# flashlight/wav2letter

Hardware: NVIDIA H100
Metric: frames_per_sec (higher is better)
Workload: dtype f32

## Files before the change

### wav2letter_b200/csrc/am_kernels.cu

```cuda
#include <cuda_runtime.h>

#include <cooperative_groups.h>

#include "common.cuh"

namespace w2l {
bool conv_mma_supported(int W, int Cin, int Cout, int K, int stride);
size_t conv_mma_arranged_floats(int Cin, int Cout, int K);
int conv_mma_fwd(cudaStream_t stream, int B, int T, int Tout, int W, int Cin, int Cout, int K, int stride, int pad_left,
                 const float* x, const float* wt, int wt_cin, int wt_cout, int flip, const float* bias, const float* add, float* y,
                 int act, float drop_p, unsigned long long seed, float* arranged, int Kfull, int tap_step, int tap_off,
                 int out_fstride, int out_foff, int out_frames);
size_t conv_mma_wgrad_parts(int B, int Tout, int W, int Cin, int Cout, int K, int stride, int* tc_out, int* per_sample_out);
int conv_mma_wgrad(cudaStream_t stream, int B, int T, int Tout, int W, int Cin, int Cout, int K, int stride, int pad_left,
                   const float* x, const float* dy, float* dwt, float* dbias, float* partial);


namespace {

constexpr int kConvRows = 4;

template <int CO, int TT>
__global__ void __launch_bounds__(96 * kConvRows) conv_time_fwd_kernel(
    int T, int Tout, int W, int Cin, int Cout, int K, int stride, int pad_left, const float* __restrict__ x,
    const float* __restrict__ wt_arranged, const float* __restrict__ bias, const float* add,
    float* y, int act, float drop_p, unsigned long long seed) {
  extern __shared__ __align__(16) float wsm[];
  const int b = blockIdx.y;
  const int w = threadIdx.x;
  const int to0 = (blockIdx.x * kConvRows + threadIdx.y) * TT;
  const int nw = Cin * K * CO;
  for (int i = threadIdx.y * blockDim.x + threadIdx.x; i < nw; i += blockDim.x * blockDim.y) wsm[i] = wt_arranged[i];
  __syncthreads();
  if (w >= W || to0 >= Tout) return;
  float acc[TT][CO];
#pragma unroll
  for (int c = 0; c < CO; ++c) {
    const float bv = (bias != nullptr && c < Cout) ? __ldg(bias + c) : 0.f;
#pragma unroll
    for (int h = 0; h < TT; ++h) acc[h][c] = bv;
  }
  const float* xb = x + (size_t)b * T * Cin * W + w;
  const size_t tstride = (size_t)Cin * W;
  for (int ci = 0; ci < Cin; ++ci) {
    const float* xc = xb + (size_t)ci * W;
    const float* wrow = wsm + (size_t)ci * K * CO;
    for (int dk = 0; dk < K; ++dk) {
      float xv[TT];
#pragma unroll
      for (int h = 0; h < TT; ++h) {
        const int tin = (to0 + h) * stride + dk - pad_left;
        xv[h] = (tin >= 0 && tin < T) ? __ldg(xc + (size_t)tin * tstride) : 0.f;
      }
      const float4* w4 = reinterpret_cast<const float4*>(wrow + dk * CO);
#pragma unroll
      for (int q = 0; q < CO / 4; ++q) {
        const float4 wv = w4[q];
#pragma unroll
        for (int h = 0; h < TT; ++h) {
          acc[h][4 * q + 0] = fmaf(xv[h], wv.x, acc[h][4 * q + 0]);
          acc[h][4 * q + 1] = fmaf(xv[h], wv.y, acc[h][4 * q + 1]);
          acc[h][4 * q + 2] = fmaf(xv[h], wv.z, acc[h][4 * q + 2]);
          acc[h][4 * q + 3] = fmaf(xv[h], wv.w, acc[h][4 * q + 3]);
        }
      }
    }
  }
  const float inv_keep = drop_p > 0.f ? 1.0f / (1.0f - drop_p) : 1.0f;
#pragma unroll
  for (int h = 0; h < TT; ++h) {
    if (to0 + h >= Tout) continue;
#pragma unroll
    for (int c = 0; c < CO; ++c) {
      if (c < Cout) {
        const size_t idx = (((size_t)b * Tout + to0 + h) * Cout + c) * W + w;
        float v = acc[h][c];
        if (act == 1) v = fmaxf(v, 0.f);
        if (drop_p > 0.f) v *= dropout_scale(seed, idx, drop_p, inv_keep);
        if (add != nullptr) v += add[idx];
        y[idx] = v;
      }
    }
  }
}

__global__ void conv_arrange_weights_kernel(int Cin, int Cout, int K, int CO, const float* __restrict__ wt,
                                            float* __restrict__ out, int flip_for_dgrad) {
  const int n_out = (flip_for_dgrad ? Cout : Cin) * K * CO;
  for (int i = blockIdx.x * blockDim.x + threadIdx.x; i < n_out; i += gridDim.x * blockDim.x) {
    const int c_inner = i % CO, dk = (i / CO) % K, c_outer = i / (CO * K);
    float v = 0.f;
    if (!flip_for_dgrad) {
      if (c_inner < Cout) v = wt[((size_t)c_inner * Cin + c_outer) * K + dk];
    } else {
      if (c_inner < Cin) v = wt[((size_t)c_outer * Cin + c_inner) * K + (K - 1 - dk)];
    }
// ... 571 lines not shown
  __syncthreads();
  int b = 0;
  for (int i = threadIdx.x; i < n_loss; i += blockDim.x) b |= !isfinite(loss[i]);
  if (b) atomicOr(&bad_loss, 1);
  __syncthreads();
  if (threadIdx.x == 0) {
    const int bad = bad_norm | bad_loss, again = retry != nullptr && bad_norm && !bad_loss;
    guard[0] = bad;
    if (bad && !again) guard[1] += 1;
    if (retry != nullptr) *retry = again;
  }
}

struct BandMasks {
  int nf, nt;
  int f0[8], f1[8], t0[8], t1[8];
};
__global__ void __launch_bounds__(256) mask_bands_kernel(long long n, int W, int CW, int T, const float* __restrict__ x, float* __restrict__ y,
                                                         BandMasks m, float val) {
  for (long long i = (long long)blockIdx.x * blockDim.x + threadIdx.x; i < n; i += (long long)gridDim.x * blockDim.x) {
    const int w = (int)(i % W), t = (int)((i / CW) % T);
    bool hit = false;
#pragma unroll
    for (int k = 0; k < 8; ++k) hit = hit || (k < m.nf && w >= m.f0[k] && w < m.f1[k]) || (k < m.nt && t >= m.t0[k] && t < m.t1[k]);
    y[i] = hit ? val : x[i];
  }
}

__global__ void transpose_bft_kernel(int F, int T, const float* __restrict__ in, float* __restrict__ out) {
  __shared__ float tile[32][33];
  const int b = blockIdx.z;
  const int t0 = blockIdx.x * 32, f0 = blockIdx.y * 32;
  const float* ib = in + (size_t)b * F * T;
  float* ob = out + (size_t)b * T * F;
  for (int j = threadIdx.y; j < 32; j += blockDim.y) {
    const int f = f0 + j, t = t0 + threadIdx.x;
    tile[j][threadIdx.x] = (f < F && t < T) ? ib[(size_t)f * T + t] : 0.f;
  }
  __syncthreads();
  for (int j = threadIdx.y; j < 32; j += blockDim.y) {
    const int t = t0 + j, f = f0 + threadIdx.x;
    if (t < T && f < F) ob[(size_t)t * F + f] = tile[threadIdx.x][j];
  }
}
template <int V>
__global__ void axpy_kernel(long long n, float a, const float* __restrict__ x, float* __restrict__ y) {
  const long long start = V * ((long long)blockIdx.x * blockDim.x + threadIdx.x), step = V * (long long)gridDim.x * blockDim.x;
#pragma unroll 2
  for (long long i = start; i < n; i += step) stv<V>(y, i, vmap([&](float xv, float yv) { return fmaf(a, xv, yv); }, ldv<V>(x, i), ldv<V>(y, i)));
}
__global__ void fill_kernel(long long n, float v, float* __restrict__ y) {
  for (long long i = (long long)blockIdx.x * blockDim.x + threadIdx.x; i < n; i += (long long)gridDim.x * blockDim.x) y[i] = v;
}
__global__ void mask_mul_kernel(long long n, const float* __restrict__ g, const float* __restrict__ ref, int mode, float scale,
                                float* __restrict__ out) {
  for (long long i = (long long)blockIdx.x * blockDim.x + threadIdx.x; i < n; i += (long long)gridDim.x * blockDim.x) {
    const float r = ref[i];
    out[i] = ((mode == 1 ? r > 0.f : r != 0.f) ? scale : 0.f) * g[i];
  }
}
__global__ void act_fwd_kernel(long long n, const float* __restrict__ x, int relu, float drop_p, unsigned long long seed,
                               float* __restrict__ y) {
  const float inv_keep = drop_p > 0.f ? 1.0f / (1.0f - drop_p) : 1.0f;
  for (long long i = (long long)blockIdx.x * blockDim.x + threadIdx.x; i < n; i += (long long)gridDim.x * blockDim.x) {
    float v = x[i];
    if (relu) v = fmaxf(v, 0.f);
    if (drop_p > 0.f) v *= dropout_scale(seed, (unsigned long long)i, drop_p, inv_keep);
    y[i] = v;
  }
}

int blocks_for(long long n, int per_block = 256 * 8) { return (int)std::min<long long>((n + per_block - 1) / per_block, sm_count() * 8); }

}
}

using namespace w2l;

static int co_pad(int c) { return (c + 3) / 4 * 4; }

static size_t conv_ws_partial_bytes(int B, int Tout, int Cin, int Cout, int K) {
  const size_t per = ((size_t)Cout * Cin * K + Cout) * sizeof(float);
  const size_t simt = (size_t)B * ((Tout + 15) / 16);
  const size_t mma = conv_mma_wgrad_parts(B, Tout, 0, Cin, Cout, K, 1, nullptr, nullptr);
  return align_up(std::max(simt, std::max(mma, (size_t)B * (size_t)std::max(Tout, 16))) * per, 256);
}
extern "C" size_t w2l_conv_time_workspace_size(int B, int Tout, int Cin, int Cout, int K) {
  const size_t arranged =
      std::max((size_t)std::max(Cin, Cout) * K * co_pad(std::max(Cin, Cout)), conv_mma_arranged_floats(Cin, Cout, K)) * sizeof(float);
  return conv_ws_partial_bytes(B, Tout, Cin, Cout, K) + align_up(arranged, 256);
}

#define W2L_CONV_DISPATCH(CO_VAL, ...)                   \
  switch (CO_VAL) {                                              \
    case 4: { constexpr int CO = 4; constexpr int TT = 8; (void)TT; __VA_ARGS__; } break;        \
    case 8: { constexpr int CO = 8; constexpr int TT = 8; (void)TT; __VA_ARGS__; } break;        \
    case 12: { constexpr int CO = 12; constexpr int TT = 8; (void)TT; __VA_ARGS__; } break;      \
    case 16: { constexpr int CO = 16; constexpr int TT = 6; (void)TT; __VA_ARGS__; } break;      \
    case 20: { constexpr int CO = 20; constexpr int TT = 4; (void)TT; __VA_ARGS__; } break;      \
    case 24: { constexpr int CO = 24; constexpr int TT = 4; (void)TT; __VA_ARGS__; } break;      \
    case 28: { constexpr int CO = 28; constexpr int TT = 3; (void)TT; __VA_ARGS__; } break;      \
    case 32: { constexpr int CO = 32; constexpr int TT = 3; (void)TT; __VA_ARGS__; } break;      \
    default: return fail(W2L_ERR_UNSUPPORTED, "conv_time: more than 32 channels is not covered"); \
  }

static int conv_check(int B, int T, int Tout, int W, int Cin, int Cout, int K, int stride) {
  if (B <= 0 || T <= 0 || Tout <= 0 || W <= 0 || Cin <= 0 || Cout <= 0 || K <= 0 || stride <= 0)
    return fail(W2L_ERR_INVALID_ARGUMENT, "conv_time: non-positive dimension");
  if (W > 80) return fail(W2L_ERR_UNSUPPORTED, "conv_time: W > 80 is not covered");
  if (Cin > 32 || Cout > 32) return fail(W2L_ERR_UNSUPPORTED, "conv_time: more than 32 channels is not covered");
  return W2L_OK;
}

extern "C" int w2l_conv_time_fwd(void* stream_, int B, int T, int Tout, int W, int Cin, int Cout, int K, int stride,
                                 int pad_left, const float* x, const float* wt, const float* bias, const float* add,
                                 float* y, int act, float dropout_p, unsigned long long seed, void* ws, size_t ws_bytes) {
  cudaStream_t stream = static_cast<cudaStream_t>(stream_);
  if (int rc = conv_check(B, T, Tout, W, Cin, Cout, K, stride)) return rc;
  if (!x || !wt || !y || !ws) return fail(W2L_ERR_INVALID_ARGUMENT, "conv_time_fwd: null pointer");
  if (ws_bytes < w2l_conv_time_workspace_size(B, Tout, Cin, Cout, K)) return fail(W2L_ERR_WORKSPACE, "conv_time_fwd: workspace too small");
  const int CO = co_pad(Cout);
  float* arranged = reinterpret_cast<float*>(static_cast<char*>(ws) + conv_ws_partial_bytes(B, Tout, Cin, Cout, K));
  if (conv_mma_supported(W, Cin, Cout, K, stride))
    return conv_mma_fwd(stream, B, T, Tout, W, Cin, Cout, K, stride, pad_left, x, wt, Cin, Cout, 0, bias, add, y, act, dropout_p, seed,
                        arranged, K, 1, 0, 1, 0, Tout);
  conv_arrange_weights_kernel<<<8, 256, 0, stream>>>(Cin, Cout, K, CO, wt, arranged, 0);
  W2L_LAUNCH_CHECK("conv_arrange_weights_kernel");
  const size_t smem = (size_t)Cin * K * CO * sizeof(float);
  dim3 block(96, kConvRows);
  W2L_CONV_DISPATCH(CO, {
    if (smem > 48 * 1024)
      W2L_CUDA_CHECK(cudaFuncSetAttribute(conv_time_fwd_kernel<CO, TT>, cudaFuncAttributeMaxDynamicSharedMemorySize, (int)smem));
    dim3 grid((Tout + kConvRows * TT - 1) / (kConvRows * TT), B);
    conv_time_fwd_kernel<CO, TT><<<grid, block, smem, stream>>>(T, Tout, W, Cin, Cout, K, stride, pad_left, x, arranged, bias, add,
                                                                y, act, dropout_p, seed);
  });
  W2L_LAUNCH_CHECK("conv_time_fwd_kernel");
  return W2L_OK;
}

extern "C" int w2l_conv_time_dgrad(void* stream_, int B, int T, int Tout, int W, int Cin, int Cout, int K, int stride,
                                   int pad_left, const float* dy, const float* wt, const float* add, float* dx, void* ws,
                                   size_t ws_bytes) {
  cudaStream_t stream = static_cast<cudaStream_t>(stream_);
  if (int rc = conv_check(B, T, Tout, W, Cin, Cout, K, stride)) return rc;
  if (!dy || !wt || !dx || !ws) return fail(W2L_ERR_INVALID_ARGUMENT, "conv_time_dgrad: null pointer");
  if (ws_bytes < w2l_conv_time_workspace_size(B, Tout, Cin, Cout, K)) return fail(W2L_ERR_WORKSPACE, "conv_time_dgrad: workspace too small");
  if (stride == 1 && conv_mma_supported(W, Cout, Cin, K, 1)) {
    float* arranged = reinterpret_cast<float*>(static_cast<char*>(ws) + conv_ws_partial_bytes(B, Tout, Cin, Cout, K));
    return conv_mma_fwd(stream, B, Tout, T, W, Cout, Cin, K, 1, K - 1 - pad_left, dy, wt, Cin, Cout, 1, nullptr, add, dx, 0, 0.f, 0ull,
                        arranged, K, 1, 0, 1, 0, T);
  }
  if (stride > 1 && stride <= K && conv_mma_supported(W, Cout, Cin, (K + stride - 1) / stride, 1)) {
    float* arranged = reinterpret_cast<float*>(static_cast<char*>(ws) + conv_ws_partial_bytes(B, Tout, Cin, Cout, K));
    for (int p = 0; p < stride; ++p) {
      const int Kp = (K - p + stride - 1) / stride;
      const int d = pad_left - p;
      const int u_min = d > 0 ? (d + stride - 1) / stride : 0;
      const int t0 = stride * u_min + p - pad_left;
      const int n_u = t0 < T ? (T - 1 - t0) / stride + 1 : 0;
      if (n_u <= 0) continue;
      if (int rc = conv_mma_fwd(stream, B, Tout, n_u, W, Cout, Cin, Kp, 1, Kp - 1 - u_min, dy, wt, Cin, Cout, 1, nullptr, add, dx, 0, 0.f, 0ull,
                                arranged, K, stride, p, stride, t0, T))
        return rc;
    }
    return W2L_OK;
  }
  if (stride == 1 && Tout == T) {
// ... 286 lines not shown
```

### wav2letter_b200/csrc/conv_mma.cu

```cuda
#include <cuda_runtime.h>

#include "common.cuh"

namespace w2l {
namespace {

constexpr int kMmaThreads = 256;

__device__ __forceinline__ float to_tf32(float x) {
  uint32_t r;
  asm("cvt.rna.tf32.f32 %0, %1;" : "=r"(r) : "f"(x));
  return __uint_as_float(r);
}
__device__ __forceinline__ float rn_tf32(float x) { return __uint_as_float((__float_as_uint(x) + 0x1000u) & 0xffffe000u); }
__device__ __forceinline__ void split_tf32(float x, float& hi, float& lo) {
  hi = rn_tf32(x);
  lo = rn_tf32(x - hi);
}
__device__ __forceinline__ void mma_tf32(float (&d)[4], const float (&a)[4], const float (&b)[2]) {
  asm volatile(
      "mma.sync.aligned.m16n8k8.row.col.f32.tf32.tf32.f32 {%0,%1,%2,%3}, {%4,%5,%6,%7}, {%8,%9}, {%0,%1,%2,%3};"
      : "+f"(d[0]), "+f"(d[1]), "+f"(d[2]), "+f"(d[3])
      : "r"(__float_as_uint(a[0])), "r"(__float_as_uint(a[1])), "r"(__float_as_uint(a[2])), "r"(__float_as_uint(a[3])),
        "r"(__float_as_uint(b[0])), "r"(__float_as_uint(b[1])));
}
template <int WT, bool kRaw = false>
__device__ __forceinline__ void stage_rows(float* dst, int pitch, const float* __restrict__ src, int W, int row_base,
                                           int rows_total, int nrows, int zero_rows) {
  constexpr int q = 2 * WT, RPW = 32 / q, kWarps = kMmaThreads / 32;
  const int warp = threadIdx.x >> 5, lane = threadIdx.x & 31;
  const int sub = lane / q, c4 = lane % q;
  if (sub < RPW) {
#pragma unroll 4
    for (int r = warp * RPW + sub; r < nrows; r += kWarps * RPW) {
      const int gr = r + row_base;
      float4 v = make_float4(0.f, 0.f, 0.f, 0.f);
      if (gr >= 0 && gr < rows_total) v = __ldg(reinterpret_cast<const float4*>(src + (size_t)gr * W) + c4);
      *reinterpret_cast<float4*>(dst + (size_t)r * pitch + 4 * c4) = kRaw ? v : make_float4(to_tf32(v.x), to_tf32(v.y), to_tf32(v.z), to_tf32(v.w));
    }
  }
  for (int i = threadIdx.x; i < zero_rows * pitch; i += blockDim.x) dst[(size_t)nrows * pitch + i] = 0.f;
}

__host__ __device__ constexpr int fwd_pitch(int WT) { return (8 * WT) % 16 == 8 ? 8 * WT : 8 * WT + 8; }
__host__ __device__ constexpr int wg_pitch(int WT) { return 8 * WT + 4; }

template <int MT, int UPW, int WT, bool kX3>
__global__ void __launch_bounds__(kMmaThreads, 2) conv_mma_fwd_kernel(int T, int Tout, int W, int Cin, int Cout, int K, int stride,
                                                                       int pad_left, int Kpad, int apitch,
                                                                       const float* __restrict__ x, const float* __restrict__ wa,
                                                                       const float* __restrict__ bias, const float* add,
                                                                       float* y, int act, float drop_p,
                                                                       unsigned long long seed, int out_fstride, int out_foff,
                                                                       int out_frames) {
  extern __shared__ __align__(16) float sm[];
  constexpr int kPitch = fwd_pitch(WT);
  constexpr int TB = 8 * UPW;
  float* xs = sm;
  const int b = blockIdx.z, w_off = blockIdx.y * 8 * WT, to0 = blockIdx.x * TB;
  const int nto = min(TB, Tout - to0);
  const int warp = threadIdx.x >> 5, lane = threadIdx.x & 31, g = lane >> 2, t4 = lane & 3;
  float acc[UPW][MT][WT][4];
#pragma unroll
  for (int u = 0; u < UPW; ++u)
#pragma unroll
    for (int m = 0; m < MT; ++m)
#pragma unroll
      for (int j = 0; j < WT; ++j)
#pragma unroll
        for (int q = 0; q < 4; ++q) acc[u][m][j][q] = 0.f;
  const int nframes = (nto - 1) * stride + K;
  stage_rows<WT, kX3>(xs, kPitch, x + (size_t)b * T * Cin * W + w_off, W, (to0 * stride - pad_left) * Cin, T * Cin, nframes * Cin, 8);
  __syncthreads();
  const float* bp[UPW];
#pragma unroll
  for (int u = 0; u < UPW; ++u) bp[u] = xs + (size_t)(min(warp + 8 * u, nto - 1) * stride * Cin + t4) * kPitch + g;
  const float* ap = wa + (size_t)g * apitch + t4;
  float a[MT][4];
#pragma unroll
  for (int m = 0; m < MT; ++m) {
    a[m][0] = __ldg(ap + (size_t)16 * m * apitch);
    a[m][1] = __ldg(ap + (size_t)(16 * m + 8) * apitch);
    a[m][2] = __ldg(ap + (size_t)16 * m * apitch + 4);
    a[m][3] = __ldg(ap + (size_t)(16 * m + 8) * apitch + 4);
  }
  for (int k0 = 0; k0 < Kpad; k0 += 8) {
    float an[MT][4];
    const int kn = min(k0 + 8, Kpad - 8);
#pragma unroll
    for (int m = 0; m < MT; ++m) {
      an[m][0] = __ldg(ap + (size_t)16 * m * apitch + kn);
      an[m][1] = __ldg(ap + (size_t)(16 * m + 8) * apitch + kn);
      an[m][2] = __ldg(ap + (size_t)16 * m * apitch + kn + 4);
      an[m][3] = __ldg(ap + (size_t)(16 * m + 8) * apitch + kn + 4);
    }
    float ah[MT][4], al[MT][4];
    if (kX3) {
#pragma unroll
      for (int m = 0; m < MT; ++m)
#pragma unroll
        for (int q = 0; q < 4; ++q) split_tf32(a[m][q], ah[m][q], al[m][q]);
    }
#pragma unroll
    for (int u = 0; u < UPW; ++u) {
      const float* bq = bp[u] + (size_t)k0 * kPitch;
#pragma unroll
      for (int j = 0; j < WT; ++j) {
        float bf[2];
        bf[0] = bq[8 * j];
        bf[1] = bq[4 * kPitch + 8 * j];
        if (kX3) {
          float bh[2], bl[2];
          split_tf32(bf[0], bh[0], bl[0]);
          split_tf32(bf[1], bh[1], bl[1]);
#pragma unroll
          for (int m = 0; m < MT; ++m) {
            mma_tf32(acc[u][m][j], al[m], bh);
            mma_tf32(acc[u][m][j], ah[m], bl);
            mma_tf32(acc[u][m][j], ah[m], bh);
          }
        } else {
#pragma unroll
          for (int m = 0; m < MT; ++m) mma_tf32(acc[u][m][j], a[m], bf);
        }
      }
    }
#pragma unroll
    for (int m = 0; m < MT; ++m)
#pragma unroll
      for (int q = 0; q < 4; ++q) a[m][q] = an[m][q];
  }
  const float inv_keep = drop_p > 0.f ? 1.0f / (1.0f - drop_p) : 1.0f;
  const bool odd = t4 & 1;
#pragma unroll
  for (int u = 0; u < UPW; ++u) {
    const int tl = warp + 8 * u;
    const int to = to0 + min(tl, nto - 1);
    const bool live = tl < nto;
#pragma unroll
    for (int m = 0; m < MT; ++m) {
#pragma unroll
      for (int hrow = 0; hrow < 2; ++hrow) {
        const int co = 16 * m + g + 8 * hrow;
        const bool ok = live && co < Cout;
        const int coc = min(co, Cout - 1);
        const float bv = bias ? __ldg(bias + coc) : 0.f;
        const size_t base = (((size_t)b * out_frames + (size_t)to * out_fstride + out_foff) * Cout + coc) * W + w_off + 2 * t4;
        float keep[WT][2];
        if (drop_p > 0.f) {
#pragma unroll
          for (int j = 0; j < WT; j += 2) {
            const int jm = (odd && j + 1 < WT) ? j + 1 : j;
            const unsigned long long idx = base + 8 * jm;
            const uint4 r = philox4x32((uint32_t)(idx >> 2), (uint32_t)(idx >> 34), (uint32_t)seed, (uint32_t)(seed >> 32));
            const uint32_t s0 = odd ? r.x : r.z, s1 = odd ? r.y : r.w;
            const uint32_t r0 = __shfl_xor_sync(0xffffffffu, s0, 1), r1 = __shfl_xor_sync(0xffffffffu, s1, 1);
            const uint32_t o0 = odd ? r.z : r.x, o1 = odd ? r.w : r.y;
            auto k = [&](uint32_t v) { return ((float)(v >> 8) * (1.0f / 16777216.0f)) >= drop_p ? inv_keep : 0.f; };
            if (j + 1 < WT) {
              keep[j][0] = odd ? k(r0) : k(o0);
              keep[j][1] = odd ? k(r1) : k(o1);
              keep[j + 1][0] = odd ? k(o0) : k(r0);
              keep[j + 1][1] = odd ? k(o1) : k(r1);
            } else {
              keep[j][0] = k(o0);
              keep[j][1] = k(o1);
            }
          }
        }
#pragma unroll
        for (int j = 0; j < WT; ++j) {
          const size_t idx = base + 8 * j;
          float v0 = acc[u][m][j][2 * hrow] + bv, v1 = acc[u][m][j][2 * hrow + 1] + bv;
          if (act == 1) {
            v0 = fmaxf(v0, 0.f);
            v1 = fmaxf(v1, 0.f);
          }
          if (drop_p > 0.f) {
            v0 *= keep[j][0];
            v1 *= keep[j][1];
          }
          if (ok) {
            if (add != nullptr) {
              const float2 av = *reinterpret_cast<const float2*>(add + idx);
              v0 += av.x;
              v1 += av.y;
            }
            *reinterpret_cast<float2*>(y + idx) = make_float2(v0, v1);
          }
        }
      }
    }
  }
}

__global__ void conv_mma_arrange_kernel(int Cin, int Cout, int Kfull, int K, int tap_step, int tap_off, int rows, int apitch,
                                        const float* __restrict__ wt, float* __restrict__ wa, int flip, int raw) {
  const int kin = flip ? Cout : Cin;
  const int mout = flip ? Cin : Cout;
  for (int i = blockIdx.x * blockDim.x + threadIdx.x; i < rows * apitch; i += gridDim.x * blockDim.x) {
    const int m = i / apitch, k = i % apitch;
    float v = 0.f;
    if (m < mout && k < K * kin) {
      const int dk = k / kin, c = k % kin;
      v = flip ? wt[((size_t)c * Cin + m) * Kfull + tap_off + tap_step * (K - 1 - dk)] : wt[((size_t)m * Cin + c) * Kfull + dk];
    }
    wa[i] = raw ? v : to_tf32(v);
  }
}

constexpr int kWgMaxNt = 8;

template <int MT, int WT, bool kX3>
__global__ void __launch_bounds__(kMmaThreads, 2) conv_mma_wgrad_kernel(int T, int Tout, int W, int Cin, int Cout, int K, int stride,
                                                                         int pad_left, int TC, int NT, const float* __restrict__ x,
                                                                         const float* __restrict__ dy, float* __restrict__ partial) {
  extern __shared__ __align__(16) float sm[];
  constexpr int kPitch = wg_pitch(WT);
  const int b = blockIdx.z, w_off = blockIdx.y * 8 * WT;
  const int Kc = K * Cin, ktiles = (Kc + 7) / 8;
  float* xs = sm;
  float* ds = sm + ((size_t)((TC - 1) * stride + K) * Cin + 8) * kPitch;
  const float* zrow = ds + (size_t)TC * Cout * kPitch;
  const int warp = threadIdx.x >> 5, lane = threadIdx.x & 31, g = lane >> 2, t4 = lane & 3;
  float acc[MT][kWgMaxNt][4];
#pragma unroll
  for (int m = 0; m < MT; ++m)
#pragma unroll
    for (int j = 0; j < kWgMaxNt; ++j)
#pragma unroll
      for (int q = 0; q < 4; ++q) acc[m][j][q] = 0.f;
  float bias_ch[4] = {0.f, 0.f, 0.f, 0.f};
  int boff[kWgMaxNt];
#pragma unroll
  for (int j = 0; j < kWgMaxNt; ++j) boff[j] = (8 * min(warp + j * (kMmaThreads / 32), ktiles - 1) + g) * kPitch + t4;
  for (int to0 = blockIdx.x * TC; to0 < Tout; to0 += gridDim.x * TC) {
    const int nto = min(TC, Tout - to0);
    const int nframes = (nto - 1) * stride + K;
    __syncthreads();
    stage_rows<WT, kX3>(xs, kPitch, x + (size_t)b * T * Cin * W + w_off, W, (to0 * stride - pad_left) * Cin, T * Cin, nframes * Cin, 8);
    stage_rows<WT, kX3>(ds, kPitch, dy + (size_t)b * Tout * Cout * W + w_off, W, to0 * Cout, Tout * Cout, nto * Cout, 0);
    if (to0 == blockIdx.x * TC)
      for (int i = threadIdx.x; i < kPitch; i += blockDim.x) ds[(size_t)TC * Cout * kPitch + i] = 0.f;
    __syncthreads();
    for (int tl = 0; tl < nto; ++tl) {
      const float* xrow = xs + (size_t)(tl * stride * Cin) * kPitch;
      const float* drow = ds + (size_t)tl * Cout * kPitch;
      const float* ar[MT][2];
#pragma unroll
      for (int m = 0; m < MT; ++m) {
        ar[m][0] = (16 * m + g < Cout ? drow + (size_t)(16 * m + g) * kPitch : zrow) + t4;
        ar[m][1] = (16 * m + g + 8 < Cout ? drow + (size_t)(16 * m + g + 8) * kPitch : zrow) + t4;
      }
#pragma unroll
      for (int wt = 0; wt < WT; ++wt) {
        float a[MT][4];
#pragma unroll
        for (int m = 0; m < MT; ++m) {
          a[m][0] = ar[m][0][8 * wt];
          a[m][1] = ar[m][1][8 * wt];
          a[m][2] = ar[m][0][8 * wt + 4];
          a[m][3] = ar[m][1][8 * wt + 4];
        }
        float ah[MT][4], al[MT][4];
        if (kX3) {
#pragma unroll
          for (int m = 0; m < MT; ++m)
#pragma unroll
            for (int q = 0; q < 4; ++q) split_tf32(a[m][q], ah[m][q], al[m][q]);
        }
#pragma unroll
        for (int j = 0; j < kWgMaxNt; ++j) {
          if (j < NT) {
            const float* bp = xrow + boff[j] + 8 * wt;
            float bf[2];
            bf[0] = bp[0];
            bf[1] = bp[4];
            if (kX3) {
              float bh[2], bl[2];
              split_tf32(bf[0], bh[0], bl[0]);
              split_tf32(bf[1], bh[1], bl[1]);
#pragma unroll
              for (int m = 0; m < MT; ++m) {
                mma_tf32(acc[m][j], al[m], bh);
                mma_tf32(acc[m][j], ah[m], bl);
                mma_tf32(acc[m][j], ah[m], bh);
              }
            } else {
#pragma unroll
              for (int m = 0; m < MT; ++m) mma_tf32(acc[m][j], a[m], bf);
            }
          }
        }
      }
    }
#pragma unroll
    for (int c = 0; c < 4; ++c) {
      const int co = warp + 8 * c;
      if (co < Cout) {
        float sacc = 0.f;
        for (int i = lane; i < nto * 8 * WT; i += 32) sacc += ds[((size_t)(i / (8 * WT)) * Cout + co) * kPitch + i % (8 * WT)];
        bias_ch[c] += sacc;
      }
    }
  }
  const size_t part = ((size_t)blockIdx.z * gridDim.y + blockIdx.y) * gridDim.x + blockIdx.x;
  float* out = partial + part * ((size_t)Cout * Cin * K + Cout);
#pragma unroll
  for (int m = 0; m < MT; ++m)
#pragma unroll
    for (int j = 0; j < kWgMaxNt; ++j) {
      const int kt = warp + j * (kMmaThreads / 32);
      if (j < NT && kt < ktiles) {
#pragma unroll
        for (int q = 0; q < 4; ++q) {
          const int co = 16 * m + g + 8 * (q >> 1), k = 8 * kt + 2 * t4 + (q & 1);
          if (co < Cout && k < Kc) {
            const int dk = k / Cin, ci = k % Cin;
            out[((size_t)co * Cin + ci) * K + dk] = acc[m][j][q];
          }
        }
      }
    }
#pragma unroll
  for (int c = 0; c < 4; ++c) {
    const int co = warp + 8 * c;
    if (co < Cout) {
      const float tot = warp_sum(bias_ch[c]);
      if (lane == 0) out[(size_t)Cout * Cin * K + co] = tot;
    }
  }
}

__global__ void __launch_bounds__(256) conv_mma_wgrad_reduce_kernel(int n_parts, int n_w, int n_b, const float* __restrict__ partial,
                                                                    float* __restrict__ dwt, float* __restrict__ dbias) {
  __shared__ float red[8][33];
  const int kx = threadIdx.x & 31, py = threadIdx.x >> 5;
  const int k = blockIdx.x * 32 + kx, n = n_w + n_b;
  float s0 = 0.f, s1 = 0.f;
  if (k < n) {
    int q = py;
    for (; q + 8 < n_parts; q += 16) {
      s0 += partial[(size_t)q * n + k];
      s1 += partial[(size_t)(q + 8) * n + k];
    }
    if (q < n_parts) s0 += partial[(size_t)q * n + k];
  }
  red[py][kx] = s0 + s1;
  __syncthreads();
  if (py == 0 && k < n) {
    float t = 0.f;
#pragma unroll
    for (int w = 0; w < 8; ++w) t += red[w][kx];
    if (k < n_w)
      dwt[k] += t;
    else if (dbias != nullptr)
      dbias[k - n_w] += t;
  }
}

int apitch_for(int Kpad) {
  int p = Kpad + 4;
  while (p % 32 != 4) ++p;
  return p;
}

}

bool conv_mma_supported(int W, int Cin, int Cout, int K, int stride) {
  return W % 8 == 0 && W <= 80 && Cin <= 32 && Cout <= 32 && K * std::max(Cin, Cout) <= 512 && stride <= K;
}
size_t conv_mma_arranged_floats(int Cin, int Cout, int K) {
  const int kin = std::max(Cin, Cout);
  const int Kpad = (K * kin + 7) / 8 * 8;
  return (size_t)32 * apitch_for(Kpad);
}
static int slice_tiles(int W) {
  for (int wt = 5; wt > 1; --wt)
    if ((W / 8) % wt == 0) return wt;
  return 1;
}
constexpr size_t kConvSmemTarget = 112 * 1024;

template <int MT, int UPW, int WT, bool kX3>
static int launch_fwd(cudaStream_t stream, dim3 grid, size_t smem, int T, int Tout, int W, int Cin, int Cout, int K, int stride,
                      int pad_left, int Kpad, int apitch, const float* x, const float* arranged, const float* bias,
                      const float* add, float* y, int act, float drop_p, unsigned long long seed, int out_fstride, int out_foff,
                      int out_frames) {
  if (smem > 48 * 1024)
    W2L_CUDA_CHECK(cudaFuncSetAttribute(conv_mma_fwd_kernel<MT, UPW, WT, kX3>, cudaFuncAttributeMaxDynamicSharedMemorySize, (int)smem));
  conv_mma_fwd_kernel<MT, UPW, WT, kX3><<<grid, kMmaThreads, smem, stream>>>(T, Tout, W, Cin, Cout, K, stride, pad_left, Kpad, apitch, x,
                                                                        arranged, bias, add, y, act, drop_p, seed, out_fstride, out_foff,
                                                                        out_frames);
  return W2L_OK;
}

int conv_mma_fwd(cudaStream_t stream, int B, int T, int Tout, int W, int Cin, int Cout, int K, int stride, int pad_left,
                 const float* x, const float* wt, int wt_cin, int wt_cout, int flip, const float* bias, const float* add, float* y,
                 int act, float drop_p, unsigned long long seed, float* arranged, int Kfull, int tap_step, int tap_off,
                 int out_fstride, int out_foff, int out_frames) {
  const int MT = (Cout + 15) / 16;
  const int Kpad = (K * Cin + 7) / 8 * 8;
  const int apitch = apitch_for(Kpad);
  const bool x3 = current_precision() == W2L_PRECISION_F32;
  conv_mma_arrange_kernel<<<16, 256, 0, stream>>>(wt_cin, wt_cout, Kfull, K, tap_step, tap_off, 16 * MT, apitch, wt, arranged, flip, x3 ? 1 : 0);
  W2L_LAUNCH_CHECK("conv_mma_arrange_kernel");
  const int WT = slice_tiles(W);
  auto bytes_for = [&](int tb) { return ((size_t)((tb - 1) * stride + K) * Cin + 8) * fwd_pitch(WT) * 4; };
  const int UPW = (MT == 1 && bytes_for(16) <= kConvSmemTarget) ? 2 : 1;
  const int TB = 8 * UPW;
  const size_t smem = bytes_for(TB);
  if (smem > 220 * 1024) return fail(W2L_ERR_UNSUPPORTED, "conv_mma_fwd: window does not fit in shared memory");
  dim3 grid((Tout + TB - 1) / TB, W / (8 * WT), B);
  int rc = W2L_OK;
#define W2L_FWD_CASE(MT_, UPW_, WT_)                                                                                  \
  if (MT == MT_ && UPW == UPW_ && WT == WT_)                                                                         \
    rc = x3 ? launch_fwd<MT_, UPW_, WT_, true>(stream, grid, smem, T, Tout, W, Cin, Cout, K, stride, pad_left, Kpad, apitch, x, arranged, \
                                               bias, add, y, act, drop_p, seed, out_fstride, out_foff, out_frames)             \
            : launch_fwd<MT_, UPW_, WT_, false>(stream, grid, smem, T, Tout, W, Cin, Cout, K, stride, pad_left, Kpad, apitch, x, arranged, \
                                                bias, add, y, act, drop_p, seed, out_fstride, out_foff, out_frames);
#define W2L_FWD_WT(WT_) W2L_FWD_CASE(1, 1, WT_) W2L_FWD_CASE(1, 2, WT_) W2L_FWD_CASE(2, 1, WT_)
  W2L_FWD_WT(1) W2L_FWD_WT(2) W2L_FWD_WT(3) W2L_FWD_WT(4) W2L_FWD_WT(5)
#undef W2L_FWD_WT
#undef W2L_FWD_CASE
  if (rc != W2L_OK) return rc;
  W2L_LAUNCH_CHECK("conv_mma_fwd_kernel");
  return W2L_OK;
}

static size_t wgrad_smem(int tc, int stride, int K, int Cin, int Cout, int WT) {
  return (((size_t)((tc - 1) * stride + K) * Cin + 8) + (size_t)tc * Cout + 1) * wg_pitch(WT) * 4;
}
static int wgrad_slice_tiles(int W, int stride, int K, int Cin, int Cout) {
  int best = 1;
  for (int wt = 5; wt >= 1; --wt) {
    if ((W / 8) % wt) continue;
    best = wt;
    if (wgrad_smem(16, stride, K, Cin, Cout, wt) <= kConvSmemTarget) return wt;
  }
  return best;
}
size_t conv_mma_wgrad_parts(int B, int Tout, int W, int Cin, int Cout, int K, int stride, int* tc_out, int* per_sample_out) {
  const int WT = W > 0 ? wgrad_slice_tiles(W, stride, K, Cin, Cout) : 1;
  const int nslices = W > 0 ? W / (8 * WT) : 10;
  int TC = 16;
  while (TC > 1 && wgrad_smem(TC, stride, K, Cin, Cout, WT) > kConvSmemTarget) TC >>= 1;
  if (tc_out) *tc_out = TC;
  const int chunks = (Tout + TC - 1) / TC;
  int per_sample = std::max(1, std::min(chunks, (2 * sm_count() + B * nslices - 1) / (B * nslices)));
  per_sample = std::max(1, std::min(per_sample, std::max(Tout, 16) / nslices));
  if (per_sample_out) *per_sample_out = per_sample;
  return (size_t)B * nslices * per_sample;
}

template <int MT, int WT, bool kX3>
static int launch_wgrad(cudaStream_t stream, dim3 grid, size_t smem, int T, int Tout, int W, int Cin, int Cout, int K, int stride,
                        int pad_left, int TC, int NT, const float* x, const float* dy, float* partial) {
  if (smem > 48 * 1024)
    W2L_CUDA_CHECK(cudaFuncSetAttribute(conv_mma_wgrad_kernel<MT, WT, kX3>, cudaFuncAttributeMaxDynamicSharedMemorySize, (int)smem));
  conv_mma_wgrad_kernel<MT, WT, kX3><<<grid, kMmaThreads, smem, stream>>>(T, Tout, W, Cin, Cout, K, stride, pad_left, TC, NT, x, dy, partial);
  return W2L_OK;
}

int conv_mma_wgrad(cudaStream_t stream, int B, int T, int Tout, int W, int Cin, int Cout, int K, int stride, int pad_left,
                   const float* x, const float* dy, float* dwt, float* dbias, float* partial) {
  const int MT = (Cout + 15) / 16;
  const int WT = wgrad_slice_tiles(W, stride, K, Cin, Cout);
  int TC = 8, per_sample = 1;
  const size_t parts = conv_mma_wgrad_parts(B, Tout, W, Cin, Cout, K, stride, &TC, &per_sample);
  const size_t smem = wgrad_smem(TC, stride, K, Cin, Cout, WT);
  if (smem > 220 * 1024) return fail(W2L_ERR_UNSUPPORTED, "conv_mma_wgrad: window does not fit in shared memory");
  const int ktiles = (K * Cin + 7) / 8, NT = (ktiles + kMmaThreads / 32 - 1) / (kMmaThreads / 32);
  if (NT > kWgMaxNt) return fail(W2L_ERR_UNSUPPORTED, "conv_mma_wgrad: filter too large for the register tiles");
  dim3 grid((unsigned)per_sample, W / (8 * WT), B);
  int rc = W2L_OK;
  const bool x3 = current_precision() == W2L_PRECISION_F32;
#define W2L_WG_CASE(MT_, WT_)                                                                                                              \
  if (MT == MT_ && WT == WT_)                                                                                                              \
    rc = x3 ? launch_wgrad<MT_, WT_, true>(stream, grid, smem, T, Tout, W, Cin, Cout, K, stride, pad_left, TC, NT, x, dy, partial)          \
            : launch_wgrad<MT_, WT_, false>(stream, grid, smem, T, Tout, W, Cin, Cout, K, stride, pad_left, TC, NT, x, dy, partial);
#define W2L_WG_WT(WT_) W2L_WG_CASE(1, WT_) W2L_WG_CASE(2, WT_)
  W2L_WG_WT(1) W2L_WG_WT(2) W2L_WG_WT(3) W2L_WG_WT(4) W2L_WG_WT(5)
#undef W2L_WG_WT
#undef W2L_WG_CASE
  if (rc != W2L_OK) return rc;
  W2L_LAUNCH_CHECK("conv_mma_wgrad_kernel");
  const int n_w = Cout * Cin * K;
  conv_mma_wgrad_reduce_kernel<<<(n_w + Cout + 31) / 32, 256, 0, stream>>>((int)parts, n_w, Cout, partial, dwt, dbias);
  W2L_LAUNCH_CHECK("conv_mma_wgrad_reduce_kernel");
  return W2L_OK;
}

}
```

Baseline: 1.024 million.

## Restructure conv weight-gradient MMA kernel with swapped operand roles and cp.async staging

Rewrites the tensor-core weight-gradient kernel so that the filter taps (K*Cin) form the M dimension and output channels form N, with each warp owning a set of M tiles. The block size now scales with the number of M tiles. Input and gradient rows are staged through cp.async in sub-steps of 8 frames instead of whole chunks. Bias partial sums are accumulated in shared memory across sub-steps, and the workspace sizing for partial results is simplified. The intent is better MMA utilisation and register tiling for larger filters, at the cost of more shared memory, more synchronisation per sub-step, and a less aggressive launch bound.

```diff
diff --git a/wav2letter_b200/csrc/am_kernels.cu b/wav2letter_b200/csrc/am_kernels.cu
--- a/wav2letter_b200/csrc/am_kernels.cu
+++ b/wav2letter_b200/csrc/am_kernels.cu
@@ -11,7 +11,7 @@
                  const float* x, const float* wt, int wt_cin, int wt_cout, int flip, const float* bias, const float* add, float* y,
                  int act, float drop_p, unsigned long long seed, float* arranged, int Kfull, int tap_step, int tap_off,
                  int out_fstride, int out_foff, int out_frames);
-size_t conv_mma_wgrad_parts(int B, int Tout, int W, int Cin, int Cout, int K, int stride, int* tc_out, int* per_sample_out);
+size_t conv_mma_wgrad_parts(int B, int Tout);
 int conv_mma_wgrad(cudaStream_t stream, int B, int T, int Tout, int W, int Cin, int Cout, int K, int stride, int pad_left,
                    const float* x, const float* dy, float* dwt, float* dbias, float* partial);
 
@@ -749,8 +749,7 @@
 static size_t conv_ws_partial_bytes(int B, int Tout, int Cin, int Cout, int K) {
   const size_t per = ((size_t)Cout * Cin * K + Cout) * sizeof(float);
   const size_t simt = (size_t)B * ((Tout + 15) / 16);
-  const size_t mma = conv_mma_wgrad_parts(B, Tout, 0, Cin, Cout, K, 1, nullptr, nullptr);
-  return align_up(std::max(simt, std::max(mma, (size_t)B * (size_t)std::max(Tout, 16))) * per, 256);
+  return align_up(std::max(simt, conv_mma_wgrad_parts(B, Tout)) * per, 256);
 }
 extern "C" size_t w2l_conv_time_workspace_size(int B, int Tout, int Cin, int Cout, int K) {
   const size_t arranged =
diff --git a/wav2letter_b200/csrc/conv_mma.cu b/wav2letter_b200/csrc/conv_mma.cu
--- a/wav2letter_b200/csrc/conv_mma.cu
+++ b/wav2letter_b200/csrc/conv_mma.cu
@@ -43,7 +43,6 @@
 }
 
 __host__ __device__ constexpr int fwd_pitch(int WT) { return (8 * WT) % 16 == 8 ? 8 * WT : 8 * WT + 8; }
-__host__ __device__ constexpr int wg_pitch(int WT) { return 8 * WT + 4; }
 
 template <int MT, int UPW, int WT, bool kX3>
 __global__ void __launch_bounds__(kMmaThreads, 2) conv_mma_fwd_kernel(int T, int Tout, int W, int Cin, int Cout, int K, int stride,
@@ -209,126 +208,140 @@
   }
 }
 
-constexpr int kWgMaxNt = 8;
-
-template <int MT, int WT, bool kX3>
-__global__ void __launch_bounds__(kMmaThreads, 2) conv_mma_wgrad_kernel(int T, int Tout, int W, int Cin, int Cout, int K, int stride,
-                                                                         int pad_left, int TC, int NT, const float* __restrict__ x,
-                                                                         const float* __restrict__ dy, float* __restrict__ partial) {
+constexpr int kWgStep = 8;
+
+__device__ __forceinline__ void cp_async16(float* dst, const float* src, bool valid) {
+  const uint32_t d = (uint32_t)__cvta_generic_to_shared(dst);
+  asm volatile("cp.async.cg.shared.global [%0], [%1], 16, %2;" ::"r"(d), "l"(src), "r"(valid ? 16 : 0) : "memory");
+}
+
+template <int MTW, int NN, bool kX3>
+__global__ void __launch_bounds__(256, MTW * NN > 6 ? 2 : 3) conv_mma_wgrad_kernel(int T, int Tout, int W, int Cin, int Cout, int K, int stride,
+                                                                int pad_left, int WT, int TC, int MW,
+                                                                const float* __restrict__ x, const float* __restrict__ dy,
+                                                                float* __restrict__ partial) {
   extern __shared__ __align__(16) float sm[];
-  constexpr int kPitch = wg_pitch(WT);
+  constexpr int NP = 8 * NN;
+  const int P = 8 * WT + 4;
+  const int q = 2 * WT;
+  const int XR = ((kWgStep - 1) * stride + K) * Cin;
+  float* xs = sm;
+  float* ds = xs + (size_t)(XR + 16) * P;
+  float* bacc = ds + (size_t)kWgStep * NP * P;
+  float* bchunk = bacc + (size_t)Cout * 32;
   const int b = blockIdx.z, w_off = blockIdx.y * 8 * WT;
-  const int Kc = K * Cin, ktiles = (Kc + 7) / 8;
-  float* xs = sm;
-  float* ds = sm + ((size_t)((TC - 1) * stride + K) * Cin + 8) * kPitch;
-  const float* zrow = ds + (size_t)TC * Cout * kPitch;
-  const int warp = threadIdx.x >> 5, lane = threadIdx.x & 31, g = lane >> 2, t4 = lane & 3;
-  float acc[MT][kWgMaxNt][4];
-#pragma unroll
-  for (int m = 0; m < MT; ++m)
-#pragma unroll
-    for (int j = 0; j < kWgMaxNt; ++j)
-#pragma unroll
-      for (int q = 0; q < 4; ++q) acc[m][j][q] = 0.f;
-  float bias_ch[4] = {0.f, 0.f, 0.f, 0.f};
-  int boff[kWgMaxNt];
-#pragma unroll
-  for (int j = 0; j < kWgMaxNt; ++j) boff[j] = (8 * min(warp + j * (kMmaThreads / 32), ktiles - 1) + g) * kPitch + t4;
+  const int Kc = K * Cin, mtiles = (Kc + 15) / 16;
+  const int nwarps = blockDim.x >> 5, warp = threadIdx.x >> 5, lane = threadIdx.x & 31, g = lane >> 2, t4 = lane & 3;
+  const int mw = warp;
+  for (int i = threadIdx.x; i < (XR + 16 + kWgStep * NP) * P + Cout * 64; i += blockDim.x) sm[i] = 0.f;
+  const float* xb = x + (size_t)b * T * Cin * W + w_off;
+  const float* dyb = dy + (size_t)b * Tout * Cout * W + w_off;
+  float acc[MTW][NN][4];
+#pragma unroll
+  for (int i = 0; i < MTW; ++i)
+#pragma unroll
+    for (int n = 0; n < NN; ++n)
+#pragma unroll
+      for (int e = 0; e < 4; ++e) acc[i][n][e] = 0.f;
   for (int to0 = blockIdx.x * TC; to0 < Tout; to0 += gridDim.x * TC) {
     const int nto = min(TC, Tout - to0);
-    const int nframes = (nto - 1) * stride + K;
-    __syncthreads();
-    stage_rows<WT, kX3>(xs, kPitch, x + (size_t)b * T * Cin * W + w_off, W, (to0 * stride - pad_left) * Cin, T * Cin, nframes * Cin, 8);
-    stage_rows<WT, kX3>(ds, kPitch, dy + (size_t)b * Tout * Cout * W + w_off, W, to0 * Cout, Tout * Cout, nto * Cout, 0);
-    if (to0 == blockIdx.x * TC)
-      for (int i = threadIdx.x; i < kPitch; i += blockDim.x) ds[(size_t)TC * Cout * kPitch + i] = 0.f;
-    __syncthreads();
-    for (int tl = 0; tl < nto; ++tl) {
-      const float* xrow = xs + (size_t)(tl * stride * Cin) * kPitch;
-      const float* drow = ds + (size_t)tl * Cout * kPitch;
-      const float* ar[MT][2];
-#pragma unroll
-      for (int m = 0; m < MT; ++m) {
-        ar[m][0] = (16 * m + g < Cout ? drow + (size_t)(16 * m + g) * kPitch : zrow) + t4;
-        ar[m][1] = (16 * m + g + 8 < Cout ? drow + (size_t)(16 * m + g + 8) * kPitch : zrow) + t4;
+    for (int s0 = 0; s0 < nto; s0 += kWgStep) {
+      const int sn = min(kWgStep, nto - s0);
+      __syncthreads();
+      const int xrows = ((sn - 1) * stride + K) * Cin, row0 = ((to0 + s0) * stride - pad_left) * Cin;
+      for (int i = threadIdx.x; i < xrows * q; i += blockDim.x) {
+        const int row = i / q, pc = i - row * q;
+        const int grow = row0 + row;
+        const bool ok = grow >= 0 && grow < T * Cin;
+        cp_async16(xs + (size_t)row * P + 4 * pc, ok ? xb + (size_t)grow * W + 4 * pc : xb, ok);
       }
-#pragma unroll
-      for (int wt = 0; wt < WT; ++wt) {
-        float a[MT][4];
-#pragma unroll
-        for (int m = 0; m < MT; ++m) {
-          a[m][0] = ar[m][0][8 * wt];
-          a[m][1] = ar[m][1][8 * wt];
-          a[m][2] = ar[m][0][8 * wt + 4];
-          a[m][3] = ar[m][1][8 * wt + 4];
-        }
-        float ah[MT][4], al[MT][4];
-        if (kX3) {
-#pragma unroll
-          for (int m = 0; m < MT; ++m)
-#pragma unroll
-            for (int q = 0; q < 4; ++q) split_tf32(a[m][q], ah[m][q], al[m][q]);
-        }
-#pragma unroll
-        for (int j = 0; j < kWgMaxNt; ++j) {
-          if (j < NT) {
-            const float* bp = xrow + boff[j] + 8 * wt;
-            float bf[2];
-            bf[0] = bp[0];
-            bf[1] = bp[4];
+      for (int i = threadIdx.x; i < sn * Cout * q; i += blockDim.x) {
+        const int row = i / q, pc = i - row * q;
+        const int tl = row / Cout, co = row - tl * Cout;
+        cp_async16(ds + (size_t)(tl * NP + co) * P + 4 * pc, dyb + ((size_t)(to0 + s0) * Cout + row) * W + 4 * pc, true);
+      }
+      asm volatile("cp.async.commit_group;" ::: "memory");
+      asm volatile("cp.async.wait_group 0;" ::: "memory");
+      __syncthreads();
+      for (int tl = 0; tl < sn; ++tl) {
+        const int base = tl * stride * Cin;
+        const float* ar[MTW][2];
+#pragma unroll
+        for (int i = 0; i < MTW; ++i) {
+          ar[i][0] = xs + (size_t)(base + 16 * (mw + MW * i) + g) * P + t4;
+          ar[i][1] = ar[i][0] + (size_t)8 * P;
+        }
+        const float* br = ds + (size_t)(tl * NP + g) * P + t4;
+        for (int wt = 0; wt < WT; ++wt) {
+          float bh[NN][2], bl[NN][2];
+#pragma unroll
+          for (int n = 0; n < NN; ++n) {
+            const float v0 = br[(size_t)8 * n * P + 8 * wt], v1 = br[(size_t)8 * n * P + 8 * wt + 4];
             if (kX3) {
-              float bh[2], bl[2];
-              split_tf32(bf[0], bh[0], bl[0]);
-              split_tf32(bf[1], bh[1], bl[1]);
-#pragma unroll
-              for (int m = 0; m < MT; ++m) {
-                mma_tf32(acc[m][j], al[m], bh);
-                mma_tf32(acc[m][j], ah[m], bl);
-                mma_tf32(acc[m][j], ah[m], bh);
+              split_tf32(v0, bh[n][0], bl[n][0]);
+              split_tf32(v1, bh[n][1], bl[n][1]);
+            } else {
+              bh[n][0] = to_tf32(v0);
+              bh[n][1] = to_tf32(v1);
+            }
+          }
+#pragma unroll
+          for (int i = 0; i < MTW; ++i) {
+            if (mw + MW * i < mtiles) {
+              float a[4];
+              a[0] = ar[i][0][8 * wt];
+              a[1] = ar[i][1][8 * wt];
+              a[2] = ar[i][0][8 * wt + 4];
+              a[3] = ar[i][1][8 * wt + 4];
+              if (kX3) {
+                float ah[4], al[4];
+#pragma unroll
+                for (int e = 0; e < 4; ++e) split_tf32(a[e], ah[e], al[e]);
+#pragma unroll
+                for (int n = 0; n < NN; ++n) {
+                  mma_tf32(acc[i][n], ah, bl[n]);
+                  mma_tf32(acc[i][n], al, bh[n]);
+                  mma_tf32(acc[i][n], ah, bh[n]);
+                }
+              } else {
+#pragma unroll
+                for (int e = 0; e < 4; ++e) a[e] = to_tf32(a[e]);
+#pragma unroll
+                for (int n = 0; n < NN; ++n) mma_tf32(acc[i][n], a, bh[n]);
               }
-            } else {
-#pragma unroll
-              for (int m = 0; m < MT; ++m) mma_tf32(acc[m][j], a[m], bf);
             }
           }
         }
       }
-    }
-#pragma unroll
-    for (int c = 0; c < 4; ++c) {
-      const int co = warp + 8 * c;
-      if (co < Cout) {
-        float sacc = 0.f;
-        for (int i = lane; i < nto * 8 * WT; i += 32) sacc += ds[((size_t)(i / (8 * WT)) * Cout + co) * kPitch + i % (8 * WT)];
-        bias_ch[c] += sacc;
+      for (int co = warp; co < Cout; co += nwarps) {
+        float sacc = s0 == 0 ? 0.f : bchunk[co * 32 + lane];
+        for (int i = lane; i < sn * 8 * WT; i += 32) {
+          const float v = ds[((size_t)(i / (8 * WT)) * NP + co) * P + i % (8 * WT)];
+          sacc += kX3 ? v : to_tf32(v);
+        }
+        bchunk[co * 32 + lane] = sacc;
       }
     }
+    for (int co = warp; co < Cout; co += nwarps) bacc[co * 32 + lane] += bchunk[co * 32 + lane];
   }
   const size_t part = ((size_t)blockIdx.z * gridDim.y + blockIdx.y) * gridDim.x + blockIdx.x;
-  float* out = partial + part * ((size_t)Cout * Cin * K + Cout);
-#pragma unroll
-  for (int m = 0; m < MT; ++m)
-#pragma unroll
-    for (int j = 0; j < kWgMaxNt; ++j) {
-      const int kt = warp + j * (kMmaThreads / 32);
-      if (j < NT && kt < ktiles) {
-#pragma unroll
-        for (int q = 0; q < 4; ++q) {
-          const int co = 16 * m + g + 8 * (q >> 1), k = 8 * kt + 2 * t4 + (q & 1);
-          if (co < Cout && k < Kc) {
-            const int dk = k / Cin, ci = k % Cin;
-            out[((size_t)co * Cin + ci) * K + dk] = acc[m][j][q];
-          }
-        }
-      }
-    }
-#pragma unroll
-  for (int c = 0; c < 4; ++c) {
-    const int co = warp + 8 * c;
-    if (co < Cout) {
-      const float tot = warp_sum(bias_ch[c]);
-      if (lane == 0) out[(size_t)Cout * Cin * K + co] = tot;
-    }
+  float* out = partial + part * ((size_t)Cout * Kc + Cout);
+#pragma unroll
+  for (int i = 0; i < MTW; ++i) {
+    const int tile = mw + MW * i;
+    if (tile < mtiles) {
+#pragma unroll
+      for (int n = 0; n < NN; ++n)
+#pragma unroll
+        for (int e = 0; e < 4; ++e) {
+          const int k = 16 * tile + g + 8 * (e >> 1), co = 8 * n + 2 * t4 + (e & 1);
+          if (k < Kc && co < Cout) out[((size_t)co * Cin + k % Cin) * K + k / Cin] = acc[i][n][e];
+        }
+    }
+  }
+  for (int co = warp; co < Cout; co += nwarps) {
+    const float tot = warp_sum(bacc[co * 32 + lane]);
+    if (lane == 0) out[(size_t)Cout * Kc + co] = tot;
   }
 }
 
@@ -428,65 +441,64 @@
   return W2L_OK;
 }
 
-static size_t wgrad_smem(int tc, int stride, int K, int Cin, int Cout, int WT) {
-  return (((size_t)((tc - 1) * stride + K) * Cin + 8) + (size_t)tc * Cout + 1) * wg_pitch(WT) * 4;
+static size_t wgrad_chunk_bytes(int tc, int stride, int K, int Cin, int Cout, int WT) {
+  return (((size_t)((tc - 1) * stride + K) * Cin + 8) + (size_t)tc * Cout + 1) * (8 * WT + 4) * 4;
 }
 static int wgrad_slice_tiles(int W, int stride, int K, int Cin, int Cout) {
   int best = 1;
   for (int wt = 5; wt >= 1; --wt) {
     if ((W / 8) % wt) continue;
     best = wt;
-    if (wgrad_smem(16, stride, K, Cin, Cout, wt) <= kConvSmemTarget) return wt;
+    if (wgrad_chunk_bytes(16, stride, K, Cin, Cout, wt) <= kConvSmemTarget) return wt;
   }
   return best;
 }
-size_t conv_mma_wgrad_parts(int B, int Tout, int W, int Cin, int Cout, int K, int stride, int* tc_out, int* per_sample_out) {
-  const int WT = W > 0 ? wgrad_slice_tiles(W, stride, K, Cin, Cout) : 1;
-  const int nslices = W > 0 ? W / (8 * WT) : 10;
+static void wgrad_partition(int B, int Tout, int W, int Cin, int Cout, int K, int stride, int* wt_out, int* tc_out, int* per_out) {
+  const int WT = wgrad_slice_tiles(W, stride, K, Cin, Cout);
+  const int nslices = W / (8 * WT);
   int TC = 16;
-  while (TC > 1 && wgrad_smem(TC, stride, K, Cin, Cout, WT) > kConvSmemTarget) TC >>= 1;
-  if (tc_out) *tc_out = TC;
+  while (TC > 1 && wgrad_chunk_bytes(TC, stride, K, Cin, Cout, WT) > kConvSmemTarget) TC >>= 1;
   const int chunks = (Tout + TC - 1) / TC;
-  int per_sample = std::max(1, std::min(chunks, (2 * sm_count() + B * nslices - 1) / (B * nslices)));
-  per_sample = std::max(1, std::min(per_sample, std::max(Tout, 16) / nslices));
-  if (per_sample_out) *per_sample_out = per_sample;
-  return (size_t)B * nslices * per_sample;
-}
-
-template <int MT, int WT, bool kX3>
-static int launch_wgrad(cudaStream_t stream, dim3 grid, size_t smem, int T, int Tout, int W, int Cin, int Cout, int K, int stride,
-                        int pad_left, int TC, int NT, const float* x, const float* dy, float* partial) {
-  if (smem > 48 * 1024)
-    W2L_CUDA_CHECK(cudaFuncSetAttribute(conv_mma_wgrad_kernel<MT, WT, kX3>, cudaFuncAttributeMaxDynamicSharedMemorySize, (int)smem));
-  conv_mma_wgrad_kernel<MT, WT, kX3><<<grid, kMmaThreads, smem, stream>>>(T, Tout, W, Cin, Cout, K, stride, pad_left, TC, NT, x, dy, partial);
+  int per = std::max(1, std::min(chunks, (2 * sm_count() + B * nslices - 1) / (B * nslices)));
+  per = std::max(1, std::min(per, std::max(Tout, 16) / nslices));
+  *wt_out = WT, *tc_out = TC, *per_out = per;
+}
+size_t conv_mma_wgrad_parts(int B, int Tout) { return (size_t)B * std::max(Tout, 16); }
+
+template <int MTW, int NN, bool kX3>
+static int launch_wgrad(cudaStream_t stream, dim3 grid, int threads, size_t smem, int T, int Tout, int W, int Cin, int Cout, int K,
+                        int stride, int pad_left, int WT, int TC, int MW, const float* x, const float* dy, float* partial) {
+  auto kern = conv_mma_wgrad_kernel<MTW, NN, kX3>;
+  if (smem > 48 * 1024) W2L_CUDA_CHECK(cudaFuncSetAttribute(kern, cudaFuncAttributeMaxDynamicSharedMemorySize, (int)smem));
+  kern<<<grid, threads, smem, stream>>>(T, Tout, W, Cin, Cout, K, stride, pad_left, WT, TC, MW, x, dy, partial);
   return W2L_OK;
 }
 
 int conv_mma_wgrad(cudaStream_t stream, int B, int T, int Tout, int W, int Cin, int Cout, int K, int stride, int pad_left,
                    const float* x, const float* dy, float* dwt, float* dbias, float* partial) {
-  const int MT = (Cout + 15) / 16;
-  const int WT = wgrad_slice_tiles(W, stride, K, Cin, Cout);
-  int TC = 8, per_sample = 1;
-  const size_t parts = conv_mma_wgrad_parts(B, Tout, W, Cin, Cout, K, stride, &TC, &per_sample);
-  const size_t smem = wgrad_smem(TC, stride, K, Cin, Cout, WT);
+  int WT = 1, TC = 16, per = 1;
+  wgrad_partition(B, Tout, W, Cin, Cout, K, stride, &WT, &TC, &per);
+  const int nslices = W / (8 * WT);
+  const int NN = (Cout + 7) / 8, mtiles = (K * Cin + 15) / 16;
+  const int MTW = std::min(4, (mtiles + 7) / 8), MW = (mtiles + MTW - 1) / MTW;
+  const size_t smem = ((size_t)(((kWgStep - 1) * stride + K) * Cin + 16 + kWgStep * 8 * NN) * (8 * WT + 4) + (size_t)Cout * 64) * sizeof(float);
   if (smem > 220 * 1024) return fail(W2L_ERR_UNSUPPORTED, "conv_mma_wgrad: window does not fit in shared memory");
-  const int ktiles = (K * Cin + 7) / 8, NT = (ktiles + kMmaThreads / 32 - 1) / (kMmaThreads / 32);
-  if (NT > kWgMaxNt) return fail(W2L_ERR_UNSUPPORTED, "conv_mma_wgrad: filter too large for the register tiles");
-  dim3 grid((unsigned)per_sample, W / (8 * WT), B);
-  int rc = W2L_OK;
+  if (MW > 8) return fail(W2L_ERR_UNSUPPORTED, "conv_mma_wgrad: filter too large for the register tiles");
+  const dim3 grid((unsigned)per, nslices, B);
   const bool x3 = current_precision() == W2L_PRECISION_F32;
-#define W2L_WG_CASE(MT_, WT_)                                                                                                              \
-  if (MT == MT_ && WT == WT_)                                                                                                              \
-    rc = x3 ? launch_wgrad<MT_, WT_, true>(stream, grid, smem, T, Tout, W, Cin, Cout, K, stride, pad_left, TC, NT, x, dy, partial)          \
-            : launch_wgrad<MT_, WT_, false>(stream, grid, smem, T, Tout, W, Cin, Cout, K, stride, pad_left, TC, NT, x, dy, partial);
-#define W2L_WG_WT(WT_) W2L_WG_CASE(1, WT_) W2L_WG_CASE(2, WT_)
-  W2L_WG_WT(1) W2L_WG_WT(2) W2L_WG_WT(3) W2L_WG_WT(4) W2L_WG_WT(5)
-#undef W2L_WG_WT
+  int rc = W2L_ERR_UNSUPPORTED;
+#define W2L_WG_CASE(MTW_, NN_)                                                                                               \
+  if (MTW == MTW_ && NN == NN_)                                                                                              \
+    rc = x3 ? launch_wgrad<MTW_, NN_, true>(stream, grid, 32 * MW, smem, T, Tout, W, Cin, Cout, K, stride, pad_left, WT, TC, MW, x, dy, partial) \
+            : launch_wgrad<MTW_, NN_, false>(stream, grid, 32 * MW, smem, T, Tout, W, Cin, Cout, K, stride, pad_left, WT, TC, MW, x, dy, partial);
+#define W2L_WG_MTW(MTW_) W2L_WG_CASE(MTW_, 1) W2L_WG_CASE(MTW_, 2) W2L_WG_CASE(MTW_, 3) W2L_WG_CASE(MTW_, 4)
+  W2L_WG_MTW(1) W2L_WG_MTW(2) W2L_WG_MTW(3) W2L_WG_MTW(4)
+#undef W2L_WG_MTW
 #undef W2L_WG_CASE
   if (rc != W2L_OK) return rc;
   W2L_LAUNCH_CHECK("conv_mma_wgrad_kernel");
   const int n_w = Cout * Cin * K;
-  conv_mma_wgrad_reduce_kernel<<<(n_w + Cout + 31) / 32, 256, 0, stream>>>((int)parts, n_w, Cout, partial, dwt, dbias);
+  conv_mma_wgrad_reduce_kernel<<<(n_w + Cout + 31) / 32, 256, 0, stream>>>((int)grid.x * grid.y * grid.z, n_w, Cout, partial, dwt, dbias);
   W2L_LAUNCH_CHECK("conv_mma_wgrad_reduce_kernel");
   return W2L_OK;
 }
```

After: 1.051 million, median of 6. 1.03x the previous value.
